# hccho2/Tacotron-Wavenet-Vocoder-Korean

Hardware: AMD Instinct MI355X
Metric: WaveNet autoregressive audio samples/sec at 24 kHz, batch=8 (higher is better)
Workload: dtype f32

## Files before the change

tacotron-wavenet-vocoder-korean_amd/csrc/twv_wavenet_xcd.hip:

```cpp
#include <hip/hip_runtime.h>
#include <stdint.h>
#include <string>
#include <type_traits>
#include "../../include/twv_amd.h"
#include "twv_layout.hpp"
#include "twv_math.hpp"
#include "twv_dev.hpp"
#include "twv_dpp.hpp"
#include "twv_categorical.hpp"
#include "twv_xcd.hpp"

using namespace twv;

#ifndef TWV_CHAIN_PAD
#define TWV_CHAIN_PAD 0
#endif
#ifndef TWV_WATCHDOG_LOG2
#define TWV_WATCHDOG_LOG2 21
#endif
#define TWV_STR2(x) #x
#define TWV_STR(x) TWV_STR2(x)
namespace {

typedef __attribute__((address_space(1))) unsigned long long gu64;
#define LDSU64(i) (((__attribute__((address_space(3))) volatile unsigned long long*)lds)[(i)])

typedef unsigned u32x2v __attribute__((ext_vector_type(2)));
typedef unsigned u32x4s __attribute__((ext_vector_type(4)));
constexpr int kAuxLoad = (int)(16u | 0x80000000u), kAuxStore = 0;
#ifndef TWV_XCD_KF
#define TWV_XCD_KF 1
#endif

__device__ __forceinline__ unsigned long long xb_load(rsrc_t rs, int uword, int lword)
{
    asm volatile("" ::: "memory");
    const u32x2v v = __builtin_amdgcn_raw_buffer_load_b64(rs, lword * 8, uword * 8, kAuxLoad);
    return ((unsigned long long)v.y << 32) | (unsigned long long)v.x;
}
__device__ __forceinline__ u32x4s xb_load2(rsrc_t rs, int uword, int lpair)
{
    asm volatile("" ::: "memory");
    return __builtin_amdgcn_raw_buffer_load_b128(rs, lpair * 16, uword * 8, kAuxLoad);
}
template <bool BAR> __device__ __forceinline__ unsigned long long xb_load_t(rsrc_t rs, int uword, int lword)
{
    if (BAR) asm volatile("" ::: "memory");
    return xb_load(rs, uword, lword);
}
__device__ __forceinline__ unsigned long long xbm_load(rsrc_t rs, int uword, int lword) { return xb_load_t<true>(rs, uword, lword); }
__device__ __forceinline__ u32x4s xbm_load2(rsrc_t rs, int uword, int lpair)
{
    asm volatile("" ::: "memory");
    return xb_load2(rs, uword, lpair);
}
__device__ __forceinline__ void xb_store(rsrc_t rs, int uword, int lword, unsigned tag, float v)
{
    __builtin_amdgcn_raw_buffer_store_b64(u32x2v{__float_as_uint(v), tag}, rs, lword * 8, uword * 8, kAuxStore);
    asm volatile("" ::: "memory");
}
__device__ __forceinline__ void xb_store2(rsrc_t rs, int uword, int lane, unsigned tag, float va, float vb)
{
    const u32x4s d = {__float_as_uint(va), tag, __float_as_uint(vb), tag};
    __builtin_amdgcn_raw_buffer_store_b128(d, rs, lane * 16, uword * 8, kAuxStore);
    asm volatile("s_nop 1" ::"v"(d) : "memory");
}
__device__ __forceinline__ unsigned g_tag(unsigned long long q) { return (unsigned)(q >> 32); }
__device__ __forceinline__ float g_val(unsigned long long q) { return __uint_as_float((unsigned)q); }

struct Poll {
    rsrc_t rs;
    int* status;
    int it;
    bool dead;
};
template <bool BAR = false>
__device__ __forceinline__ bool poll_tick(Poll& p, int code)
{
    if (p.dead) return false;
    if (((++p.it) & 63) == 0) {
        if (xb_load_t<BAR>(p.rs, (int)XcdExch::CTRL + 1, 0) != 0ull) { p.dead = true; return false; }
        if (p.it > (1 << TWV_WATCHDOG_LOG2)) {
            atomicMax(p.status, code);
            xb_store(p.rs, (int)XcdExch::CTRL + 1, 0, 1u, 0.0f);
            p.dead = true;
            return false;
        }
    }
    return true;
}
__device__ __forceinline__ void nap_until(unsigned long long target)
{
#pragma nounroll
    for (int i = 0; i < 4096 && __builtin_amdgcn_s_memtime() < target; ++i) __builtin_amdgcn_s_sleep(8);
}

__device__ __forceinline__ unsigned lds_byte_addr_u64(int i)
{
    return (unsigned)(unsigned long)(&((__attribute__((address_space(3))) unsigned long long*)lds)[i]);
}
__device__ __forceinline__ unsigned lds_byte_addr_u32(int i)
{
    return (unsigned)(unsigned long)(&((__attribute__((address_space(3))) unsigned*)lds)[i]);
}
enum { SPIN_EQ = 0, SPIN_GE = 1 };
#define TWV_SPIN_TAIL                 \
    "s_cmp_eq_u64 vcc, exec\n"        \
    "s_cbranch_scc1 2f\n"             \
    "s_sub_u32 %1, %1, 1\n"           \
    "s_cmp_lg_u32 %1, 0\n"            \
    "s_cbranch_scc1 1b\n"             \
    "2:"
template <int CMP>
__device__ __forceinline__ unsigned long long lds_spin_tag(unsigned byte_addr, unsigned tag, unsigned looks, unsigned& left)
{
    unsigned long long q;
    unsigned n;
    if (CMP == SPIN_GE) {
        const unsigned long long need = (unsigned long long)tag << 32;
        asm volatile(
            "s_mov_b32 %1, %4\n"
            "1:\n"
            "ds_read_b64 %0, %2\n"
            "s_waitcnt lgkmcnt(0)\n"
            "v_cmp_le_u64 vcc, %3, %0\n"
            TWV_SPIN_TAIL
            : "=&v"(q), "=&s"(n)
            : "v"(byte_addr), "s"(need), "s"(looks)
            : "vcc", "scc", "memory");
    } else {
        unsigned long long d;
        const unsigned long long want = (unsigned long long)tag;
        asm volatile(
            "s_mov_b32 %1, %5\n"
            "1:\n"
            "ds_read_b64 %0, %3\n"
            "s_waitcnt lgkmcnt(0)\n"
            "v_lshrrev_b64 %2, 32, %0\n"
            "v_cmp_eq_u64 vcc, %4, %2\n"
            TWV_SPIN_TAIL
            : "=&v"(q), "=&s"(n), "=&v"(d)
            : "v"(byte_addr), "s"(want), "s"(looks)
            : "vcc", "scc", "memory");
    }
    left = n;
    return q;
}
__device__ __forceinline__ void lds_spin_count(unsigned byte_addr, unsigned need, unsigned looks, unsigned& left)
{
    unsigned c, n;
    asm volatile(
        "s_mov_b32 %1, %4\n"
        "1:\n"
        "ds_read_b32 %0, %2\n"
        "s_waitcnt lgkmcnt(0)\n"
        "v_cmp_le_u32 vcc, %3, %0\n"
        TWV_SPIN_TAIL
        : "=&v"(c), "=&s"(n)
        : "v"(byte_addr), "s"(need), "s"(looks)
        : "vcc", "scc", "memory");
    left = n;
}
__device__ __forceinline__ unsigned tag_diff_acc(unsigned acc, unsigned got, unsigned tag)
{
    asm("v_xad_u32 %0, %1, %2, %0" : "+v"(acc) : "v"(got), "s"(tag));
    return acc;
}
template <int CMP>
__device__ __forceinline__ unsigned long long xb_spin_tag(rsrc_t rs, int uword, int lword, unsigned tag, unsigned looks, unsigned& left)
{
    unsigned long long q;
    unsigned n;
    if (CMP == SPIN_GE) {
        const unsigned long long need = (unsigned long long)tag << 32;
        asm volatile(
            "s_mov_b32 %1, %6\n"
            "1:\n"
            "buffer_load_dwordx2 %0, %2, %3, %4 offen sc0 sc1\n"
            "s_waitcnt vmcnt(0)\n"
            "v_cmp_le_u64 vcc, %5, %0\n"
            TWV_SPIN_TAIL
            : "=&v"(q), "=&s"(n)
            : "v"(lword * 8), "s"(rs), "s"(uword * 8), "s"(need), "s"(looks)
            : "vcc", "scc", "memory");
    } else {
        unsigned long long d;
        const unsigned long long want = (unsigned long long)tag;
        asm volatile(
            "s_mov_b32 %1, %7\n"
            "1:\n"
            "buffer_load_dwordx2 %0, %3, %4, %5 offen sc0 sc1\n"
            "s_waitcnt vmcnt(0)\n"
            "v_lshrrev_b64 %2, 32, %0\n"
            "v_cmp_eq_u64 vcc, %6, %2\n"
            TWV_SPIN_TAIL
            : "=&v"(q), "=&s"(n), "=&v"(d)
            : "v"(lword * 8), "s"(rs), "s"(uword * 8), "s"(want), "s"(looks)
            : "vcc", "scc", "memory");
    }
    left = n;
    return q;
}

__device__ __forceinline__ int lane_of_z(int k) { return ((k & 2) ? 16 : 0) + 2 * (k >> 2) + (k & 1); }
__device__ __forceinline__ int lane_of_x(int j) { return j < 16 ? j : 16 + j; }

struct ChainRegs { float wc[32]; float bd; };
__device__ __forceinline__ void dot32_dpp_chain_lo(const float (&w)[16], float xa, float init, float (&c)[4])
{
    float c0 = init, c1, c2, c3;
    asm volatile(
        "s_nop 1\n" TWV_ALIGN8
        "v_fmac_f32_dpp %0, %4, %5 row_newbcast:0 row_mask:0xf bank_mask:0xf\n"
        "v_mul_f32_dpp %1, %4, %6 row_newbcast:1 row_mask:0xf bank_mask:0xf\n"
        "v_mul_f32_dpp %2, %4, %7 row_newbcast:2 row_mask:0xf bank_mask:0xf\n"
        "v_mul_f32_dpp %3, %4, %8 row_newbcast:3 row_mask:0xf bank_mask:0xf\n"
        "v_fmac_f32_dpp %0, %4, %9 row_newbcast:4 row_mask:0xf bank_mask:0xf\n"
        "v_fmac_f32_dpp %1, %4, %10 row_newbcast:5 row_mask:0xf bank_mask:0xf\n"
        "v_fmac_f32_dpp %2, %4, %11 row_newbcast:6 row_mask:0xf bank_mask:0xf\n"
        "v_fmac_f32_dpp %3, %4, %12 row_newbcast:7 row_mask:0xf bank_mask:0xf\n"
        "v_fmac_f32_dpp %0, %4, %13 row_newbcast:8 row_mask:0xf bank_mask:0xf\n"
        "v_fmac_f32_dpp %1, %4, %14 row_newbcast:9 row_mask:0xf bank_mask:0xf\n"
        "v_fmac_f32_dpp %2, %4, %15 row_newbcast:10 row_mask:0xf bank_mask:0xf\n"
        "v_fmac_f32_dpp %3, %4, %16 row_newbcast:11 row_mask:0xf bank_mask:0xf\n"
        "v_fmac_f32_dpp %0, %4, %17 row_newbcast:12 row_mask:0xf bank_mask:0xf\n"
        "v_fmac_f32_dpp %1, %4, %18 row_newbcast:13 row_mask:0xf bank_mask:0xf\n"
        "v_fmac_f32_dpp %2, %4, %19 row_newbcast:14 row_mask:0xf bank_mask:0xf\n"
        "v_fmac_f32_dpp %3, %4, %20 row_newbcast:15 row_mask:0xf bank_mask:0xf"
        : "+v"(c0), "=&v"(c1), "=&v"(c2), "=&v"(c3)
        : "v"(xa), "v"(w[0]), "v"(w[1]), "v"(w[2]), "v"(w[3]), "v"(w[4]), "v"(w[5]), "v"(w[6]), "v"(w[7]), "v"(w[8]), "v"(w[9]), "v"(w[10]), "v"(w[11]), "v"(w[12]), "v"(w[13]), "v"(w[14]), "v"(w[15]));
    c[0] = c0; c[1] = c1; c[2] = c2; c[3] = c3;
}
__device__ __forceinline__ float dot32_dpp_chain_hi(const float (&w)[16], float xb, const float (&c)[4])
{
    float c0 = c[0], c1 = c[1], c2 = c[2], c3 = c[3];
    asm volatile(
        TWV_ALIGN8
        "v_fmac_f32_dpp %0, %4, %5 row_newbcast:0 row_mask:0xf bank_mask:0xf\n"
        "v_fmac_f32_dpp %1, %4, %6 row_newbcast:1 row_mask:0xf bank_mask:0xf\n"
        "v_fmac_f32_dpp %2, %4, %7 row_newbcast:2 row_mask:0xf bank_mask:0xf\n"
        "v_fmac_f32_dpp %3, %4, %8 row_newbcast:3 row_mask:0xf bank_mask:0xf\n"
        "v_fmac_f32_dpp %0, %4, %9 row_newbcast:4 row_mask:0xf bank_mask:0xf\n"
        "v_fmac_f32_dpp %1, %4, %10 row_newbcast:5 row_mask:0xf bank_mask:0xf\n"
        "v_fmac_f32_dpp %2, %4, %11 row_newbcast:6 row_mask:0xf bank_mask:0xf\n"
        "v_fmac_f32_dpp %3, %4, %12 row_newbcast:7 row_mask:0xf bank_mask:0xf\n"
        "v_fmac_f32_dpp %0, %4, %13 row_newbcast:8 row_mask:0xf bank_mask:0xf\n"
        "v_fmac_f32_dpp %1, %4, %14 row_newbcast:9 row_mask:0xf bank_mask:0xf\n"
        "v_fmac_f32_dpp %2, %4, %15 row_newbcast:10 row_mask:0xf bank_mask:0xf\n"
        "v_fmac_f32_dpp %3, %4, %16 row_newbcast:11 row_mask:0xf bank_mask:0xf\n"
        "v_fmac_f32_dpp %0, %4, %17 row_newbcast:12 row_mask:0xf bank_mask:0xf\n"
        "v_fmac_f32_dpp %1, %4, %18 row_newbcast:13 row_mask:0xf bank_mask:0xf\n"
        "v_fmac_f32_dpp %2, %4, %19 row_newbcast:14 row_mask:0xf bank_mask:0xf\n"
        "v_fmac_f32_dpp %3, %4, %20 row_newbcast:15 row_mask:0xf bank_mask:0xf"
        : "+v"(c0), "+v"(c1), "+v"(c2), "+v"(c3)
        : "v"(xb), "v"(w[0]), "v"(w[1]), "v"(w[2]), "v"(w[3]), "v"(w[4]), "v"(w[5]), "v"(w[6]), "v"(w[7]), "v"(w[8]), "v"(w[9]), "v"(w[10]), "v"(w[11]), "v"(w[12]), "v"(w[13]), "v"(w[14]), "v"(w[15]));
    return (c0 + c1) + (c2 + c3);
}

#define XSTAMP(cond_, slot_) do { if ((INSTR & 1) && a.prof != nullptr && b == a.prof_stream && t < a.prof_steps && lane == 0 && (cond_)) a.prof[(long long)t * 64 + (slot_)] = wall_clock64(); } while (0)

#define WACC_DECL() unsigned long long wacc_[6] = {0, 0, 0, 0, 0, 0}, w0_ = 0, wt0_ = 0; if (INSTR & 4) wt0_ = __builtin_amdgcn_s_memtime()
#define WACC_T0() do { if (INSTR & 4) w0_ = __builtin_amdgcn_s_memtime(); } while (0)
#define WACC_T1(i_) do { if (INSTR & 4) wacc_[i_] += __builtin_amdgcn_s_memtime() - w0_; } while (0)
constexpr int kTraceStep = 2000;
#define WTRACE(cond_, slot_) do { if ((INSTR & 4) && a.prof != nullptr && t == kTraceStep && (cond_) && lane == 0) a.prof[2048 + (slot_)] = wall_clock64(); } while (0)
#define WACC_OUT(prof_, slot_, wave_) do { if ((INSTR & 4) && (prof_) != nullptr && (slot_) >= 0 && lane == 0) {                 \
        unsigned long long* o_ = (prof_) + (((slot_) * 8 + (wave_)) * 8);                                                        \
        o_[0] = __builtin_amdgcn_s_memtime() - wt0_;                                                                             \
        o_[1] = wacc_[0]; o_[2] = wacc_[1]; o_[3] = wacc_[2]; o_[4] = wacc_[3]; o_[5] = wacc_[4]; o_[6] = wacc_[5]; } } while (0)
#define XMARK(role_, stage_) do { if ((INSTR & 1) && lane == 0) xb_store(rs, (int)XcdExch::MARK + (role_) * 8 + (int)(threadIdx.x >> 6), 0, (unsigned)t + 1u, (float)(stage_)); } while (0)

enum { ROLE_CHAIN = 0, ROLE_SERVICE = 1, ROLE_SKIP0 = 2, ROLE_CONV0 = 10 };
constexpr int kXcdStreamsPerXcd = kXcdStreams / 8;

struct XArgs {
    XcdLaunch p;
    int n_lc_wg, lc_lpw;
    int n_conv1;
    int total_roles;
};

template <int NS> struct XStreams { rsrc_t rs[NS]; int b[NS]; };
__device__ __forceinline__ rsrc_t exch_rsrc(const XcdLaunch& a, int b)
{
    return __builtin_amdgcn_make_buffer_rsrc(a.exch + (long long)b * XcdExch::WORDS, 0, (int)(XcdExch::WORDS * 8), 0x00020000);
}
struct XLazyRs { const XcdLaunch* a; int xcc, ns; __device__ __forceinline__ rsrc_t operator[](int k) const { return exch_rsrc(*a, xcc + 8 * (k < ns ? k : 0)); } };
struct XLazyB { int xcc, ns; __device__ __forceinline__ int operator[](int k) const { return xcc + 8 * (k < ns ? k : 0); } };
template <int NS> struct XStreamsLazy { XLazyRs rs; XLazyB b; };
constexpr int kSkipLdsWords = 32 * 64;
constexpr int kConvLdsFloats = 16 * 64 + 64;

constexpr int kChainLpw = 5;
template <int INSTR, bool ALL, bool FORCED, bool SEG1, bool TWOSEG, int NC, bool ONEHOT = false, bool HEAD = false, bool CONT = false>
__device__ __forceinline__ void chain_role(const XArgs& xa, int b, rsrc_t rs, const unsigned looks)
{
    const XcdLaunch& a = xa.p;
    const Layout& L = a.lay;
    const int w = __builtin_amdgcn_readfirstlane(threadIdx.x >> 6), lane = threadIdx.x & 63;
    const int NL = L.NL, T = a.T;
    const bool use_bias = L.use_bias != 0, has_gc = L.G > 0, has_lc = L.L > 0;
    constexpr bool forced = FORCED;
    constexpr int kLayerWaves = kXcdSeg0Layers / kChainLpw;
    const int l0 = (SEG1 ? kXcdSeg0Layers : 0) + kChainLpw * w;
    const int lw0 = kChainLpw * w;
    const int cap = (HEAD || w >= kLayerWaves) ? 0 : kChainLpw;
    int nl = NL - l0;
    nl = nl < 0 ? 0 : (nl > cap ? cap : nl);
    const int nlc = NC >= 0 ? NC : nl;
    const bool next_has = (l0 + nl < NL);
    constexpr bool head = HEAD;
    const bool to_seg1 = TWOSEG && !SEG1 && w == kLayerWaves - 1 && next_has;
    constexpr bool two_seg = TWOSEG;
    if (nl == 0 && !head) return;
    const int oc = dpp_conv_out(lane), od = dpp_dense_out(lane);
    const ActCoef coef = act_coef(lane >= 32);
    float* stb = a.state + (long long)b * L.state_stride;
    Poll pl{rs, a.status, 0, false};
    constexpr int O_WD = 2048;
    constexpr int O_WH = kXcdChainHalfTiles;

    float wlo[kChainLpw - 1][16], whi[kChainLpw][16], bdi[kChainLpw];
#pragma unroll
    for (int i = 0; i < kChainLpw; ++i) {
        if (!HEAD && i < nl) {
            const f32x4* src = reinterpret_cast<const f32x4*>(a.P + L.off_xl + (long long)(l0 + i) * kXcdXlFloats) + lane;
#pragma unroll
            for (int q = 0; q < 4; ++q) {
                const f32x4 lo = src[q * 64], hi = src[(4 + q) * 64];
                if (i == 0) LDS4((O_WH >> 2) + (w * 4 + q) * 64 + lane) = lo;
                else { wlo[i > 0 ? i - 1 : 0][4 * q] = lo.x; wlo[i > 0 ? i - 1 : 0][4 * q + 1] = lo.y; wlo[i > 0 ? i - 1 : 0][4 * q + 2] = lo.z; wlo[i > 0 ? i - 1 : 0][4 * q + 3] = lo.w; }
                whi[i][4 * q] = hi.x; whi[i][4 * q + 1] = hi.y; whi[i][4 * q + 2] = hi.z; whi[i][4 * q + 3] = hi.w;
            }
#pragma unroll
            for (int q = 0; q < 4; ++q) LDS4((O_WD >> 2) + ((lw0 + i) * 4 + q) * 64 + lane) = src[(8 + q) * 64];
            const f32x4 v = src[12 * 64];
            bdi[i] = dense_bias_init(lane, use_bias ? v.y : 0.0f);
        }
    }
    float wcz[32];
    float ha = 0.0f, hb = 0.0f, first_in = 0.0f, b2v = 0.0f, s_lnl = 0.0f, s_tq = 0.0f, samp = 0.0f;
    float cp[4] = {0.0f, 0.0f, 0.0f, 0.0f};
    int q_prev = 0, q_valid = 0, samp_q = 0, first_q = 0;
    float w0row = 0.0f;
    double u_next = 0.0;
    const int chx = dpp_dense_out(lane);
    const bool sampler = head && !forced;
    const bool is15 = (lane & 15) == 15;
    auto causal_prepare = [&]() {
        const float t1 = __int_as_float(__builtin_amdgcn_update_dpp(0, __float_as_int(ha), 0x101, 0xf, 0xf, true));
        const float b0 = __int_as_float(__builtin_amdgcn_update_dpp(0, __float_as_int(hb), 0x150, 0xf, 0xf, true));
        ha = is15 ? b0 : t1;
        hb = __int_as_float(__builtin_amdgcn_update_dpp(0, __float_as_int(hb), 0x101, 0xf, 0xf, true));
        causal_partial_dpp(wcz, ha, hb, cp);
    };
    auto noise = [&](int t) {
        const float* up = a.uniforms + ((long long)b * T + t) * (L.nr_mix + 1);
        const float u = lane <= L.nr_mix ? up[lane] : 0.5f;
        s_lnl = log_e(-log_e(u));
        const float uu = __shfl(u, L.nr_mix);
        s_tq = log_e(uu) - log_e(1.0f - uu);
    };
    if (head) {
        if constexpr (ONEHOT) {
            const int* meta = reinterpret_cast<const int*>(stb + L.st_meta);
            q_valid = __builtin_amdgcn_readfirstlane(meta[M_PREV_VALID]);
            q_prev = __builtin_amdgcn_readfirstlane(meta[M_QPREV]) & (L.Q - 1);
            w0row = a.P[L.off_causal + (long long)q_prev * 32 + chx];
            if (!forced) first_q = reinterpret_cast<const int*>(a.first_input)[b];
        } else {
            const f32x4* src = reinterpret_cast<const f32x4*>(a.P + L.off_xc) + lane;
#pragma unroll
            for (int q = 0; q < 8; ++q) { const f32x4 v = src[q * 64]; wcz[4 * q] = v.x; wcz[4 * q + 1] = v.y; wcz[4 * q + 2] = v.z; wcz[4 * q + 3] = v.w; }
            ha = stb[L.st_hist + (lane & 15)];
            hb = stb[L.st_hist + 16 + (lane & 15)];
            if (!forced) first_in = reinterpret_cast<const float*>(a.first_input)[b];
            if (sampler && use_bias && lane < L.O) b2v = a.P[L.off_b2 + lane];
            causal_prepare();
        }
    }
    __builtin_amdgcn_s_waitcnt(0);
    asm volatile(".p2align 6\n\t.rept " TWV_STR(TWV_CHAIN_PAD) "\n\ts_nop 0\n\t.endr" ::: "memory");

    float X = 0.0f;
    unsigned long long t_in = 0, in_period = 0, now_in = 0;
    unsigned long long t_tab = 0, tab_period = 0, now_tab = 0;
    for (int t = 0; t < T && !pl.dead; ++t) {
        asm volatile(".p2align 6");
        const unsigned tag = (unsigned)t + 1u;
        if (head) {
            if (forced && t > 0) {
                unsigned left = 0;
                if (two_seg) (void)xb_spin_tag<SPIN_EQ>(rs, (int)XcdExch::DONE, lane, (unsigned)t, looks, left);
                else (void)lds_spin_tag<SPIN_EQ>(lds_byte_addr_u64(8 * 64 + lane), (unsigned)t, looks, left);
                if (__builtin_expect(left == 0, 0)) {
                    pl.it = 0;
                    for (;;) {
                        const unsigned long long q = two_seg ? xb_load(rs, (int)XcdExch::DONE, lane) : LDSU64(8 * 64 + lane);
                        if (__all(g_tag(q) == (unsigned)t)) break;
                        if (!poll_tick(pl, 35)) break;
                        __builtin_amdgcn_s_sleep(2);
                    }
                }
                if (pl.dead) break;
            }
            XSTAMP(true, 0);
            if constexpr (ONEHOT) {
                const int q_raw = forced ? reinterpret_cast<const int*>(a.forced)[(long long)b * T + t] : (t == 0 ? first_q : samp_q);
                const int q_in = __builtin_amdgcn_readfirstlane(q_raw) & (L.Q - 1);
                const float w1row = a.P[L.off_causal + ((long long)L.Q + q_in) * 32 + chx];
                const float x0 = q_valid ? w0row + w1row : w1row;
                LDSU64(0 * 64 + lane) = ((unsigned long long)tag << 32) | (unsigned long long)__float_as_uint(x0);
                XSTAMP(true, 1);
                if (lane == 0) {
                    if (sampler && t > 0) reinterpret_cast<int*>(a.out)[(long long)b * T + t - 1] = samp_q;
                    xb_store(rs, (int)XcdExch::CTRL, 0, tag, 0.0f);
                }
                q_prev = q_in; q_valid = 1;
                w0row = a.P[L.off_causal + (long long)q_in * 32 + chx];
                if (sampler) u_next = reinterpret_cast<const double*>(a.uniforms)[(long long)b * T + t];
            } else {
            const float s_in = forced ? reinterpret_cast<const float*>(a.forced)[(long long)b * T + t] : (t == 0 ? first_in : samp);
            const float c3 = fma_(wcz[31], s_in, cp[3]);
            const float x0 = (cp[0] + cp[1]) + (cp[2] + c3);
            LDSU64(0 * 64 + lane) = ((unsigned long long)tag << 32) | (unsigned long long)__float_as_uint(x0);
            XSTAMP(true, 1);
            if (lane == 0) {
                if (sampler && t > 0) a.out[(long long)b * T + t - 1] = samp;
                xb_store(rs, (int)XcdExch::CTRL, 0, tag, 0.0f);
            }
            hb = is15 ? s_in : hb;
            if (t + 1 < T) causal_prepare();
            if (sampler) noise(t);
            }
            if (sampler) {
                const unsigned long long d = now_tab - t_tab;
                tab_period = (t_tab != 0 && d < (1ull << 18)) ? d : 0;
                t_tab = now_tab;
            }
            __builtin_amdgcn_s_setprio(0);
        }
        XMARK(SEG1 ? 30 : ROLE_CHAIN, 1);
        float pre[kChainLpw] = {0.0f, 0.0f, 0.0f, 0.0f, 0.0f};
        float w0lo[16];
        if (nlc > 0) {
            pl.it = 0;
            for (;;) {
                bool ok = true;
#pragma unroll
                for (int i = 0; i < kChainLpw; ++i) {
                    if (i < nlc) {
                        const unsigned long long qp = xb_load(rs, (int)XcdExch::PG + (l0 + i) * 64, oc);
                        ok = ok && g_tag(qp) == tag;
                        pre[i] = g_val(qp);
                    }
                }
                if (__all(ok)) break;
                if (!poll_tick(pl, 31)) break;
                __builtin_amdgcn_s_sleep(4);
            }
            XSTAMP(!SEG1, 26 + w);
            XMARK(SEG1 ? 30 : ROLE_CHAIN, 2);
            if (in_period) nap_until(t_in + in_period - (in_period >> 4));
            asm volatile("" ::: "memory");
#pragma unroll
            for (int k = 0; k < 4; ++k) {
                const f32x4 v = LDS4((O_WH >> 2) + (w * 4 + k) * 64 + lane);
                w0lo[4 * k] = v.x; w0lo[4 * k + 1] = v.y; w0lo[4 * k + 2] = v.z; w0lo[4 * k + 3] = v.w;
            }
// ... 114 lines not shown
            if (tab_period) nap_until(t_tab + tab_period - (tab_period >> 3));
            __builtin_amdgcn_s_setprio(3);
            const int half = lane >> 5;
            unsigned long long q[8];
            pl.it = 0;
            for (;;) {
                unsigned diff = 0;
#pragma unroll
                for (int k = 0; k < 4; ++k) {
                    const u32x4s d = xb_load2(rs, (int)XcdExch::PT, (half * 4 + k) * 32 + (lane & 31));
                    q[2 * k] = ((unsigned long long)d.y << 32) | d.x;
                    q[2 * k + 1] = ((unsigned long long)d.w << 32) | d.z;
                    diff = tag_diff_acc(tag_diff_acc(diff, d.y, tag), d.w, tag);
                }
                if (__all(diff == 0u)) break;
                if (!poll_tick(pl, 34)) break;
            }
            now_tab = __builtin_amdgcn_s_memtime();
            XSTAMP(true, 18);
            XMARK(SEG1 ? 30 : ROLE_CHAIN, 5);
            float y = g_val(q[0]);
#pragma unroll
            for (int k = 1; k < 8; ++k) y = y + g_val(q[k]);
#pragma unroll
            for (int k = 0; k < 8; ++k) {
                const auto sw = __builtin_amdgcn_permlane32_swap((unsigned)q[k], (unsigned)q[k], false, false);
                y = y + __uint_as_float(sw[1]);
            }
            if (use_bias && lane < L.O) y = y + b2v;
            if ((INSTR & 2) && a.dbg != nullptr && t < a.dbg_steps)
                a.dbg[((long long)b * a.dbg_steps + t) * ((long long)NL * 64 + L.Opad) + (long long)NL * 64 + lane] = y;
            const int nr = L.nr_mix;
            const float lsmin = (float)-32.23619130191664;
            const float e_all = exp_e(y > lsmin ? y : lsmin);
            const float ninf = __uint_as_float(0xff800000u);
            const float gmb = (lane < nr) ? y - s_lnl : ninf;
            float mx = gmb;
            mx = fmaxf(mx, __int_as_float(__builtin_amdgcn_update_dpp(__float_as_int(ninf), __float_as_int(mx), 0x111, 0xf, 0xf, false)));
            mx = fmaxf(mx, __int_as_float(__builtin_amdgcn_update_dpp(__float_as_int(ninf), __float_as_int(mx), 0x112, 0xf, 0xf, false)));
            mx = fmaxf(mx, __int_as_float(__builtin_amdgcn_update_dpp(__float_as_int(ninf), __float_as_int(mx), 0x114, 0xf, 0xf, false)));
            mx = fmaxf(mx, __int_as_float(__builtin_amdgcn_update_dpp(__float_as_int(ninf), __float_as_int(mx), 0x118, 0xf, 0xf, false)));
            const float best = __int_as_float(__builtin_amdgcn_readlane(__float_as_int(mx), 15));
            const unsigned long long hit = __ballot(lane < nr && gmb == best);
            const int k = hit ? (int)__ffsll((long long)hit) - 1 : 0;
            const float mean = __int_as_float(__builtin_amdgcn_readlane(__float_as_int(y), nr + k));
            const float e = __int_as_float(__builtin_amdgcn_readlane(__float_as_int(e_all), 2 * nr + k));
            const float prod = e * s_tq;
            float xs = mean + prod;
            xs = xs > -1.0f ? xs : -1.0f;
            xs = xs < 1.0f ? xs : 1.0f;
            samp = xs;
            XSTAMP(true, 19);
        }
    }

    if (head) {
        if constexpr (ONEHOT) {
            if (lane == 0) {
                if (sampler && !pl.dead && T > 0) reinterpret_cast<int*>(a.out)[(long long)b * T + T - 1] = samp_q;
                int* meta = reinterpret_cast<int*>(stb + L.st_meta);
                meta[M_TABS] = meta[M_TABS] + T;
                meta[M_PREV_VALID] = q_valid;
                meta[M_QPREV] = q_prev;
            }
        } else {
        if (sampler && !pl.dead && T > 0 && lane == 0) a.out[(long long)b * T + T - 1] = samp;
        if (lane < 16) stb[L.st_hist + lane] = ha;
        else if (lane < 32) stb[L.st_hist + lane] = hb;
        if (lane == 0) {
            int* meta = reinterpret_cast<int*>(stb + L.st_meta);
            meta[M_TABS] = meta[M_TABS] + T;
        }
        }
    }
}

#define TWV_FMAC16_DPP(c0, c1, c2, c3, x, w)                                                          \
    asm volatile(                                                                                      \
        "s_nop 1\n" TWV_ALIGN8                                                                         \
        "v_fmac_f32_dpp %0, %4, %5 row_newbcast:0 row_mask:0xf bank_mask:0xf\n"                        \
        "v_fmac_f32_dpp %1, %4, %6 row_newbcast:1 row_mask:0xf bank_mask:0xf\n"                        \
        "v_fmac_f32_dpp %2, %4, %7 row_newbcast:2 row_mask:0xf bank_mask:0xf\n"                        \
        "v_fmac_f32_dpp %3, %4, %8 row_newbcast:3 row_mask:0xf bank_mask:0xf\n"                        \
        "v_fmac_f32_dpp %0, %4, %9 row_newbcast:4 row_mask:0xf bank_mask:0xf\n"                        \
        "v_fmac_f32_dpp %1, %4, %10 row_newbcast:5 row_mask:0xf bank_mask:0xf\n"                       \
        "v_fmac_f32_dpp %2, %4, %11 row_newbcast:6 row_mask:0xf bank_mask:0xf\n"                       \
        "v_fmac_f32_dpp %3, %4, %12 row_newbcast:7 row_mask:0xf bank_mask:0xf\n"                       \
        "v_fmac_f32_dpp %0, %4, %13 row_newbcast:8 row_mask:0xf bank_mask:0xf\n"                       \
        "v_fmac_f32_dpp %1, %4, %14 row_newbcast:9 row_mask:0xf bank_mask:0xf\n"                       \
        "v_fmac_f32_dpp %2, %4, %15 row_newbcast:10 row_mask:0xf bank_mask:0xf\n"                      \
        "v_fmac_f32_dpp %3, %4, %16 row_newbcast:11 row_mask:0xf bank_mask:0xf\n"                      \
        "v_fmac_f32_dpp %0, %4, %17 row_newbcast:12 row_mask:0xf bank_mask:0xf\n"                      \
        "v_fmac_f32_dpp %1, %4, %18 row_newbcast:13 row_mask:0xf bank_mask:0xf\n"                      \
        "v_fmac_f32_dpp %2, %4, %19 row_newbcast:14 row_mask:0xf bank_mask:0xf\n"                      \
        "v_fmac_f32_dpp %3, %4, %20 row_newbcast:15 row_mask:0xf bank_mask:0xf"                        \
        : "+v"(c0), "+v"(c1), "+v"(c2), "+v"(c3)                                                       \
        : "v"(x), "v"(w[0]), "v"(w[1]), "v"(w[2]), "v"(w[3]), "v"(w[4]), "v"(w[5]), "v"(w[6]), "v"(w[7]), "v"(w[8]), "v"(w[9]), \
          "v"(w[10]), "v"(w[11]), "v"(w[12]), "v"(w[13]), "v"(w[14]), "v"(w[15]))
__device__ __forceinline__ float dot32_dpp_lds(int off4, int lane, float xa, float xb)
{
    float c0 = 0.0f, c1 = 0.0f, c2 = 0.0f, c3 = 0.0f;
#pragma unroll
    for (int h = 0; h < 2; ++h) {
        float w[16];
#pragma unroll
        for (int kq = 0; kq < 4; ++kq) {
            const f32x4 q = LDS4(off4 + (4 * h + kq) * 64 + lane);
            w[4 * kq + 0] = q.x; w[4 * kq + 1] = q.y; w[4 * kq + 2] = q.z; w[4 * kq + 3] = q.w;
        }
        if (h == 0) { TWV_FMAC16_DPP(c0, c1, c2, c3, xa, w); }
        else { TWV_FMAC16_DPP(c0, c1, c2, c3, xb, w); }
    }
    return (c0 + c1) + (c2 + c3);
}
__device__ __forceinline__ void copy_tile_to_lds(int off4, const float* base, int lane)
{
    const f32x4* p = reinterpret_cast<const f32x4*>(base) + lane;
#pragma unroll
    for (int kq = 0; kq < 8; ++kq) LDS4(off4 + kq * 64 + lane) = p[kq * 64];
}

__device__ __forceinline__ unsigned ring_slot(unsigned pos0, unsigned t, unsigned d)
{
    const unsigned v = pos0 + t;
    return (d & (d - 1)) == 0 ? (v & (d - 1)) : v % d;
}
template <int INSTR, bool BIG>
__device__ __forceinline__ void service_role(const XArgs& xa, int b, rsrc_t rs)
{
    const XcdLaunch& a = xa.p;
    const Layout& L = a.lay;
    const int s = __builtin_amdgcn_readfirstlane(threadIdx.x >> 6), lane = threadIdx.x & 63;
    const int NL = L.NL, T = a.T;
    const bool has_lc = L.L > 0, use_bias = L.use_bias != 0, has_gc = L.G > 0;
    float* stb = a.state + (long long)b * L.state_stride;
    float* ring = stb + L.st_ring;
    const int* pmeta = reinterpret_cast<const int*>(a.P + L.off_meta);
    int* ringpos = reinterpret_cast<int*>(stb + L.st_ringpos);
    Poll pl{rs, a.status, 0, false};
    constexpr int kReg = 4, kLds = BIG ? 3 : 0, kSlots = kReg + kLds;
    const int NLDS = BIG ? (NL > 8 * kReg ? NL - 8 * kReg : 0) : 0;
    int nown = 0, nlds = 0;
#pragma unroll
    for (int i = 0; i < kReg; ++i) if (NLDS + s + 8 * i < NL) nown = i + 1;
#pragma unroll
    for (int j = 0; j < kLds; ++j) if (s + 8 * j < NLDS) nlds = j + 1;
    if (nown == 0 && nlds == 0) return;
    Tile t0[kReg];
    unsigned dil[kSlots], roff[kSlots], pos0[kSlots];
    int lay_of[kSlots];
    float bfg[kSlots], gcv[kSlots];
#pragma unroll
    for (int i = 0; i < kSlots; ++i) {
        dil[i] = 1; roff[i] = 0; pos0[i] = 0; bfg[i] = 0.0f; gcv[i] = 0.0f;
        const bool is_lds = i < kLds;
        const int l = is_lds ? s + 8 * i : NLDS + s + 8 * (i - kLds);
        const bool have = is_lds ? i < nlds : (i - kLds) < nown;
        lay_of[i] = have ? l : -1;
        if (have) {
            const float* src = a.P + L.off_layer0 + (long long)l * L.layer_stride + LayerOff::T0;
            if (is_lds) copy_tile_to_lds(l * (kTile / 4), src, lane);
            else load_tile(t0[i - kLds < 0 ? 0 : i - kLds], src, lane);
            dil[i] = (unsigned)pmeta[l]; roff[i] = (unsigned)pmeta[64 + l]; pos0[i] = (unsigned)ringpos[l];
            if (use_bias) bfg[i] = a.P[L.off_layer0 + (long long)l * L.layer_stride + LayerOff::BFG + lane];
            if (has_gc) gcv[i] = a.cond[XH_WORDS + ((long long)b * NL + l) * 64 + lane];
        }
    }
    auto addend = [&](int i, float pre, float lcv) __attribute__((always_inline)) -> float {
        float v = pre;
        if (use_bias) v = v + bfg[i];
        if (has_gc) v = v + gcv[i];
        if (has_lc) v = v + lcv;
        return v;
    };
    const int n16 = lane & 15;
    auto tap0 = [&](int i, unsigned t, float& xa_, float& xb_) __attribute__((always_inline)) {
        const unsigned slot = ring_slot(pos0[i], t, dil[i]);
        const unsigned long long* p = reinterpret_cast<const unsigned long long*>(ring + roff[i] + slot * 32);
        const unsigned long long qa = __hip_atomic_load((gu64*)(p + (n16 >> 1)), __ATOMIC_RELAXED, __HIP_MEMORY_SCOPE_AGENT);
        const unsigned long long qb = __hip_atomic_load((gu64*)(p + 8 + (n16 >> 1)), __ATOMIC_RELAXED, __HIP_MEMORY_SCOPE_AGENT);
        xa_ = __uint_as_float((n16 & 1) ? (unsigned)(qa >> 32) : (unsigned)qa);
        xb_ = __uint_as_float((n16 & 1) ? (unsigned)(qb >> 32) : (unsigned)qb);
    };
    auto dot_slot = [&](int i, float oa, float ob) __attribute__((always_inline)) -> float {
        if (i < kLds) return dot32_dpp_lds(lay_of[i] * (kTile / 4), lane, oa, ob);
        return dot32_dpp(t0[i - kLds < 0 ? 0 : i - kLds].w, oa, ob);
    };
#pragma unroll
    for (int i = 0; i < kSlots; ++i) {
        if (lay_of[i] >= 0) {
            const int l = lay_of[i];
            float xa_, xb_;
            tap0(i, 0u, xa_, xb_);
            const float pre = dot_slot(i, xa_, xb_);
            const float lcv = has_lc ? stb[L.st_lcprev + l * 64 + lane] : 0.0f;
            xb_store(rs, (int)XcdExch::PG + l * 64, lane, 1u, addend(i, pre, lcv));
        }
    }
    for (int t = 0; t < T && !pl.dead; ++t) {
        asm volatile(".p2align 6");
        const unsigned tag = (unsigned)t + 1u;
#pragma unroll
        for (int i = 0; i < kSlots; ++i) {
            if (lay_of[i] >= 0 && !pl.dead) {
                const int l = lay_of[i];
                const bool more = t + 1 < T;
                float oa = 0.0f, ob = 0.0f;
                if (more && dil[i] > 1) tap0(i, (unsigned)t + 1u, oa, ob);
                XMARK(ROLE_SERVICE, 10 + i);
                unsigned long long qa, qb;
                pl.it = 0;
                for (;;) {
                    qa = xb_load(rs, (int)XcdExch::ZX + l * 128 + 1, n16 * 2);
                    qb = xb_load(rs, (int)XcdExch::ZX + l * 128 + 65, n16 * 2);
                    if (__all(g_tag(qa) == tag && g_tag(qb) == tag)) break;
                    if (!poll_tick(pl, 41)) break;
                    __builtin_amdgcn_s_sleep(8);
                }
                if (pl.dead) break;
                const float xa_ = g_val(qa), xb_ = g_val(qb);
                const unsigned slot = ring_slot(pos0[i], (unsigned)t, dil[i]);
                if (lane < 32) ring[roff[i] + slot * 32 + lane] = lane < 16 ? xa_ : xb_;
                if (more) {
                    if (dil[i] == 1) { oa = xa_; ob = xb_; }
                    const float pre = dot_slot(i, oa, ob);
                    float lcv = 0.0f;
                    XMARK(ROLE_SERVICE, 20 + i);
                    if (has_lc) {
                        const int lw = (int)XcdExch::LCR + (((t + 1) % kXcdLcRing) * kXcdLs + l) * 64;
                        unsigned long long ql;
                        pl.it = 0;
                        for (;;) {
                            ql = xb_load(rs, lw, lane);
                            if (__all(g_tag(ql) == tag + 1u)) break;
                            if (!poll_tick(pl, 42)) break;
                            __builtin_amdgcn_s_sleep(8);
                        }
                        if (pl.dead) break;
                        lcv = g_val(ql);
                    }
                    xb_store(rs, (int)XcdExch::PG + l * 64, lane, tag + 1u, addend(i, pre, lcv));
                }
            }
        }
    }
    if (lane == 0 && !pl.dead) {
#pragma unroll
        for (int i = 0; i < kSlots; ++i)
            if (lay_of[i] >= 0) ringpos[lay_of[i]] = (int)((pos0[i] + (unsigned)T) % dil[i]);
    }
}

template <int INSTR, int NS, bool BIG, int KF = 0>
__device__ __forceinline__ void skip_role(const XArgs& xa, const XStreams<NS>& sx, int g, const unsigned looks)
{
    const XcdLaunch& a = xa.p;
    const Layout& L = a.lay;
    const int v = __builtin_amdgcn_readfirstlane(threadIdx.x >> 6), lane = threadIdx.x & 63;
    const int NL = L.NL - KF, T = a.T;
    const bool use_bias = L.use_bias != 0;
    Poll pl{sx.rs[0], a.status, 0, false};
    constexpr int kReg = BIG ? 5 : 4, kLds = BIG ? 2 : 0, kSlots = kReg + kLds;
    const int NLDS = BIG ? (NL > 8 * kReg ? NL - 8 * kReg : 0) : 0;
    const int SW = BIG ? NL * 64 : kSkipLdsWords;
    const int o_tile4 = (NS * SW * 2 + 3) >> 2;
    int nown = 0, nlds = 0;
#pragma unroll
    for (int i = 0; i < kReg; ++i) if (NLDS + v + 8 * i < NL) nown = i + 1;
#pragma unroll
    for (int j = 0; j < kLds; ++j) if (v + 8 * j < NLDS) nlds = j + 1;
    if (nown == 0 && nlds == 0) return;
    Tile ws[kReg];
    float bs[kSlots];
#pragma unroll
    for (int i = 0; i < kSlots; ++i) bs[i] = 0.0f;
#pragma unroll
    for (int i = 0; i < kReg; ++i) {
        if (i < nown) {
            const long long lb = L.off_layer0 + (long long)(NLDS + v + 8 * i) * L.layer_stride;
            load_tile(ws[i], a.P + lb + LayerOff::SK + (long long)g * kTile, lane);
            if (use_bias) bs[kLds + i] = a.P[lb + LayerOff::SK + (long long)L.NSJ * kTile + g * 64 + lane];
        }
    }
#pragma unroll
    for (int j = 0; j < kLds; ++j) {
        if (j < nlds) {
            const long long lb = L.off_layer0 + (long long)(v + 8 * j) * L.layer_stride;
            copy_tile_to_lds(o_tile4 + (v + 8 * j) * (kTile / 4), a.P + lb + LayerOff::SK + (long long)g * kTile, lane);
            if (use_bias) bs[j] = a.P[lb + LayerOff::SK + (long long)L.NSJ * kTile + g * 64 + lane];
        }
    }
    const int n16 = lane & 15;
    const int zc_lane = lane_of_z((lane < 32 ? 0 : 16) + n16);
    unsigned long long seen[kSlots], period = 0;
#pragma unroll
    for (int i = 0; i < kSlots; ++i) seen[i] = 0;
    for (int t = 0; t < T && !pl.dead; ++t) {
        asm volatile(".p2align 6");
        const unsigned tag = (unsigned)t + 1u;
        auto own_layer = [&](auto&& dot, const float bias, const int l, const int si) __attribute__((always_inline)) {
            {
                if (period) nap_until(seen[si] + period - (period >> 3));
                const bool last = l == NL - 1;
                const int lp = l > 0 ? l - 1 : 0;
#pragma unroll
                for (int k = 0; k < NS; ++k) {
                    if (pl.dead) break;
                    const rsrc_t rs = sx.rs[k];
                    const int b = sx.b[k];
                    pl.rs = rs;
                    XMARK(ROLE_SKIP0 + g, 10 + si);
                    unsigned long long qz, qp = 0;
                    pl.it = 0;
                    if (last) {
                        unsigned left = 0;
                        qz = xb_spin_tag<SPIN_EQ>(rs, (int)XcdExch::ZX + l * 128, zc_lane * 2, tag, looks, left);
                        if (__builtin_expect(left == 0, 0)) {
                            pl.it = 0;
                            for (;;) {
                                qz = xb_load(rs, (int)XcdExch::ZX + l * 128, zc_lane * 2);
                                if (__all(g_tag(qz) == tag)) break;
                                if (!poll_tick(pl, 51)) break;
                            }
                        }
                        qp = LDSU64(k * SW + lp * 64 + lane);
                    } else
                    for (;;) {
                        qz = xb_load(rs, (int)XcdExch::ZX + l * 128, zc_lane * 2);
                        qp = LDSU64(k * SW + lp * 64 + lane);
                        if (__all(g_tag(qz) == tag)) break;
                        if (!poll_tick(pl, 51)) break;
                        __builtin_amdgcn_s_sleep(1);
                    }
                    if ((INSTR & 1) && pl.dead && g == 0 && lane == 0) {
                        xb_store(rs, (int)XcdExch::MARK + 176 + v * 4, 0, g_tag(qz), __uint_as_float(g_tag(qz)));
                        xb_store(rs, (int)XcdExch::MARK + 177 + v * 4, 0, (unsigned)l, __uint_as_float((unsigned)pl.it));
                        xb_store(rs, (int)XcdExch::MARK + 178 + v * 4, 0, tag, __uint_as_float((unsigned)si));
                    }
                    XSTAMP(g == 0 && last, 20);
                    const auto sw = __builtin_amdgcn_permlane32_swap((unsigned)qz, (unsigned)qz, false, false);
                    float val = dot(__uint_as_float(sw[0]), __uint_as_float(sw[1]));
                    if (use_bias) val = val + bias;
                    float tot = val;
                    if (l > 0) {
                        asm volatile("" : "+v"(val));
                        if (!__all(g_tag(qp) == tag)) {
                            unsigned left = 0;
                            qp = lds_spin_tag<SPIN_GE>(lds_byte_addr_u64(k * SW + lp * 64 + lane), tag, looks, left);
                            if (left == 0) {
                                pl.it = 0;
                                while (!__all(g_tag(qp) == tag)) {
                                    if (!poll_tick(pl, 52)) break;
                                    qp = LDSU64(k * SW + lp * 64 + lane);
                                }
                            }
                        }
                        tot = g_val(qp) + val;
                    }
                    if (pl.dead) break;
                    if (last) {
                        const float h = (KF > 0 || tot > 0.0f) ? tot : 0.0f;
                        xb_store(rs, (int)XcdExch::H1 + g * 64, lane, tag, h);
                        XSTAMP(g == 0, 21);
                    } else {
                        LDSU64(k * SW + l * 64 + lane) = ((unsigned long long)tag << 32) | (unsigned long long)__float_as_uint(tot);
                    }
                    if (k == 0) {
                        const unsigned long long now = __builtin_amdgcn_s_memtime();
                        if (si == 0) { const unsigned long long d = now - seen[0]; period = (seen[0] != 0 && d < (1ull << 18)) ? d : 0; }
                        seen[si] = now;
                    }
                }
            }
        };
#pragma unroll
        for (int j = 0; j < kLds; ++j) {
            if (j < nlds && !pl.dead)
                own_layer([&](float xa_, float xb_) __attribute__((always_inline)) { return dot32_dpp_lds(o_tile4 + (v + 8 * j) * (kTile / 4), lane, xa_, xb_); }, bs[j], v + 8 * j, j);
        }
#pragma unroll
        for (int i = 0; i < kReg; ++i) {
            if (i < nown && !pl.dead)
                own_layer([&](float xa_, float xb_) __attribute__((always_inline)) { return dot32_dpp(ws[i].w, xa_, xb_); }, bs[kLds + i], NLDS + v + 8 * i, kLds + i);
        }
    }
    if (pl.dead && lane == 0) {
#pragma unroll
        for (int k = 0; k < NS; ++k) xb_store(sx.rs[k], (int)XcdExch::CTRL + 1, 0, 1u, 0.0f);
    }
}

template <int KF, bool BAR>
__device__ __forceinline__ unsigned long long conv1_fetch_h1(Poll& pl, const rsrc_t rs, const int v, const int lane, const unsigned tag, const int last_layer,
                                                             const int zc_lane, const float (&wl)[32], const float bl, const bool use_bias, bool& saw_z, const unsigned looks)
{
    unsigned long long q;
    pl.it = 0;
    if (KF > 0) {
        unsigned long long qz;
        float val = 0.0f;
        for (;;) {
            qz = xb_load_t<BAR>(rs, (int)XcdExch::ZX + last_layer * 128, zc_lane * 2);
            q = xb_load_t<BAR>(rs, (int)XcdExch::H1 + v * 64, lane);
            if (__all(g_tag(qz) == tag)) {
                const auto sw = __builtin_amdgcn_permlane32_swap((unsigned)qz, (unsigned)qz, false, false);
                val = dot32_dpp(wl, __uint_as_float(sw[0]), __uint_as_float(sw[1]));
                if (use_bias) val = val + bl;
                saw_z = true;
                break;
            }
            if (!poll_tick<BAR>(pl, 61)) break;
            __builtin_amdgcn_s_sleep(1);
        }
        if (saw_z && !__all(g_tag(q) == tag)) {
            unsigned left = 0;
            q = xb_spin_tag<SPIN_EQ>(rs, (int)XcdExch::H1 + v * 64, lane, tag, looks, left);
            if (__builtin_expect(left == 0, 0)) {
                pl.it = 0;
                for (;;) {
                    q = xb_load_t<BAR>(rs, (int)XcdExch::H1 + v * 64, lane);
                    if (__all(g_tag(q) == tag)) break;
                    if (!poll_tick<BAR>(pl, 61)) break;
                }
            }
        }
        const float tot = g_val(q) + val;
        const float h = tot > 0.0f ? tot : 0.0f;
        q = (unsigned long long)__float_as_uint(h);
    } else {
        for (;;) {
            q = xb_load_t<BAR>(rs, (int)XcdExch::H1 + v * 64, lane);
            if (__all(g_tag(q) == tag)) break;
            if (!poll_tick<BAR>(pl, 61)) break;
            __builtin_amdgcn_s_sleep(1);
        }
    }
    return q;
}
__device__ __forceinline__ void conv1_load_last_skip(const XcdLaunch& a, const int v, const int lane, Tile& wl, float& bl)
{
    const Layout& L = a.lay;
    const long long lb = L.off_layer0 + (long long)(L.NL - 1) * L.layer_stride;
    load_tile(wl, a.P + lb + LayerOff::SK + (long long)v * kTile, lane);
    if (L.use_bias != 0) bl = a.P[lb + LayerOff::SK + (long long)L.NSJ * kTile + v * 64 + lane];
}
__device__ __forceinline__ void load_half_tile(float (&w)[16], const float* base, const int obase, const int lane)
{
    const float2* p = reinterpret_cast<const float2*>(base + (obase + dpp_dense_out(lane)) * 4 + (((lane >> 4) & 1) ? 2 : 0));
#pragma unroll
    for (int j = 0; j < 8; ++j) {
        const float2 q = p[j * 128];
        w[2 * j] = q.x; w[2 * j + 1] = q.y;
    }
}
__device__ __forceinline__ float conv1d2_chunk_dpp(const float (&t2)[16], const float h)
{
    const float s = dot16_dpp(t2, h);
    const auto ds = __builtin_amdgcn_permlane16_swap(__float_as_uint(s), __float_as_uint(s), false, false);
    return __uint_as_float(ds[0]) + __uint_as_float(ds[1]);
}

template <int INSTR, int NS, bool BAR = false, class SX = XStreams<NS>, int KF = 0>
__device__ __forceinline__ void conv1_role(const XArgs& xa, const SX& sx, int g, const int ns_rt, const int prof_slot, const unsigned looks)
{
    const XcdLaunch& a = xa.p;
    const Layout& L = a.lay;
    const int v = __builtin_amdgcn_readfirstlane(threadIdx.x >> 6), lane = threadIdx.x & 63;
    const int T = a.T, NCH = L.NCH;
    const bool use_bias = L.use_bias != 0;
    Poll pl{sx.rs[0], a.status, 0, false};
    constexpr int O_PART = 0, O_CNT = 16 * 64;
    if (threadIdx.x < NS) LDSI(threadIdx.x * kConvLdsFloats + O_CNT) = 0;
    __syncthreads();
    const int c0 = 2 * v, c1 = 2 * v + 1;
    Tile ta, tb;
    load_tile(ta, a.P + L.off_w1 + ((long long)g * NCH + c0) * kTile, lane);
    load_tile(tb, a.P + L.off_w1 + ((long long)g * NCH + c1) * kTile, lane);
    const bool summer = v < 2;
    const int hz = 32 * v + dpp_z_index(lane);
    float b1v = 0.0f;
    float t2[16];
    if (summer) {
        if (use_bias) b1v = a.P[L.off_b1 + g * 64 + hz];
        load_half_tile(t2, a.P + L.off_w2 + (long long)(2 * g + v) * kTile, 0, lane);
    }
    Tile wl;
    float bl = 0.0f;
    if (KF > 0) conv1_load_last_skip(a, v, lane, wl, bl);
    const int zc_lane = lane_of_z((lane < 32 ? 0 : 16) + (lane & 15));
    unsigned long long t_arr = 0, period = 0;
    WACC_DECL();
    for (int t = 0; t < T && !pl.dead; ++t) {
        asm volatile(".p2align 6");
        const unsigned tag = (unsigned)t + 1u;
        WACC_T0();
        if (period) nap_until(t_arr + period - (period >> 3));
        WACC_T1(0);
#pragma unroll
        for (int k = 0; k < NS; ++k) {
            if (pl.dead) break;
            if (k >= ns_rt) break;
            const rsrc_t rs = sx.rs[k];
            const int b = sx.b[k];
            const int ob = k * kConvLdsFloats;
            pl.rs = rs;
            XMARK(ROLE_CONV0 + g, 1);
            WACC_T0();
            bool saw_z = false;
            const unsigned long long q = conv1_fetch_h1<KF, BAR>(pl, rs, v, lane, tag, L.NL - 1, zc_lane, wl.w, bl, use_bias, saw_z, looks);
            (void)saw_z;
            WACC_T1(1);
            WTRACE(prof_slot >= 0 && k == 0, 400 + g * 8 + v);
            unsigned long long now_arr = 0;
            if (k == 0) now_arr = __builtin_amdgcn_s_memtime();
            XSTAMP(g == 0 && v == 0, 22);
            const unsigned hq = (unsigned)q;
            const auto p16 = __builtin_amdgcn_permlane16_swap(hq, hq, false, false);
            const auto pa = __builtin_amdgcn_permlane32_swap(p16[0], p16[0], false, false);
            const auto pb = __builtin_amdgcn_permlane32_swap(p16[1], p16[1], false, false);
            float r0, r1;
            dot32_dpp_x2(ta.w, __uint_as_float(pa[0]), __uint_as_float(pb[0]), tb.w, __uint_as_float(pa[1]), __uint_as_float(pb[1]), r0, r1);
            lds[ob + O_PART + c0 * 64 + lane] = r0;
            lds[ob + O_PART + c1 * 64 + lane] = r1;
            asm volatile("" ::: "memory");
            if (lane == 0) __hip_atomic_fetch_add(&LDSI(ob + O_CNT), 1, __ATOMIC_RELAXED, __HIP_MEMORY_SCOPE_WORKGROUP);
            if (k == 0) {
                const unsigned long long d = now_arr - t_arr;
                period = (t_arr != 0 && d < (1ull << 18)) ? d : 0;
                t_arr = now_arr;
            }
            XSTAMP(g == 0 && v == 0, 23);
            XMARK(ROLE_CONV0 + g, 2);
            if (summer) {
                WACC_T0();
                unsigned left = 0;
                if (!BAR) lds_spin_count(lds_byte_addr_u32(ob + O_CNT), 8u * tag, looks, left);
                if (__builtin_expect(left == 0, 0)) {
                    pl.it = 0;
                    while (LDSVI(ob + O_CNT) < 8 * (t + 1)) { if (!poll_tick<BAR>(pl, 62)) break; }
                }
                WACC_T1(2);
                asm volatile("" ::: "memory");
                XSTAMP(g == 0 && v == 0, 24);
                float cp[16];
#pragma unroll
                for (int ch = 0; ch < 16; ++ch) cp[ch] = lds[ob + O_PART + ch * 64 + hz];
                __builtin_amdgcn_sched_barrier(0);
                float r = cp[0];
#pragma unroll
                for (int ch = 1; ch < 16; ++ch) r = r + cp[ch];
                if (use_bias) r = r + b1v;
                const float h = r > 0.0f ? r : 0.0f;
                const float p = conv1d2_chunk_dpp(t2, h);
                if ((lane & 16) == 0) xb_store(rs, (int)XcdExch::PT, (g * 32 + dpp_dense_out(lane)) * 2 + v, tag, p);
                WTRACE(prof_slot >= 0 && k == 0, 480 + g * 2 + v);
                XSTAMP(g == 0 && v == 0, 25);
            }
        }
    }
    if (pl.dead && lane == 0) {
#pragma unroll
        for (int k = 0; k < NS; ++k) xb_store(sx.rs[k], (int)XcdExch::CTRL + 1, 0, 1u, 0.0f);
    }
    WACC_OUT(a.prof, prof_slot, v);
}

template <int INSTR, int KF>
__device__ __forceinline__ void conv1_half_role(const XArgs& xa, const XStreams<1>& sx, const int g, const int hh, const unsigned looks)
{
    static_assert(KF > 0, "the last layer's skip 1x1 runs here");
    const XcdLaunch& a = xa.p;
    const Layout& L = a.lay;
    const int v = __builtin_amdgcn_readfirstlane(threadIdx.x >> 6), lane = threadIdx.x & 63;
    const int T = a.T, NCH = L.NCH;
    const bool use_bias = L.use_bias != 0;
    const rsrc_t rs = sx.rs[0];
    const int b = sx.b[0];
    Poll pl{rs, a.status, 0, false};
    constexpr int O_PART = 0, O_CNT = 16 * 64;
    if (threadIdx.x == 0) LDSI(O_CNT) = 0;
    __syncthreads();
    const int c0 = 2 * v, c1 = 2 * v + 1;
    float ta[16], tb[16];
    load_half_tile(ta, a.P + L.off_w1 + ((long long)g * NCH + c0) * kTile, 32 * hh, lane);
    load_half_tile(tb, a.P + L.off_w1 + ((long long)g * NCH + c1) * kTile, 32 * hh, lane);
    const int zi = dpp_z_index(lane), od = dpp_dense_out(lane);
    const int hl = 32 * (lane >> 5) + zi;
    const bool summer = v == 0;
    float b1v = 0.0f;
    float t2[16];
    if (summer) {
        if (use_bias) b1v = a.P[L.off_b1 + g * 64 + 32 * hh + zi];
        load_half_tile(t2, a.P + L.off_w2 + (long long)(2 * g + hh) * kTile, 0, lane);
    }
    Tile wl;
    float bl = 0.0f;
    conv1_load_last_skip(a, v, hl, wl, bl);
    const int zc_lane = lane_of_z((lane < 32 ? 0 : 16) + (lane & 15));
    unsigned long long t_arr = 0, period = 0;
    for (int t = 0; t < T && !pl.dead; ++t) {
        asm volatile(".p2align 6");
        const unsigned tag = (unsigned)t + 1u;
        if (period) nap_until(t_arr + period - (period >> 3));
        XMARK(ROLE_CONV0 + 2 * g + hh, 1);
        bool saw_z = false;
        const unsigned long long q = conv1_fetch_h1<KF, false>(pl, rs, v, hl, tag, L.NL - 1, zc_lane, wl.w, bl, use_bias, saw_z, looks);
        (void)saw_z;
        const unsigned long long now_arr = __builtin_amdgcn_s_memtime();
        XSTAMP(g == 0 && hh == 0 && v == 0, 22);
        const unsigned hq = (unsigned)q;
        const auto hs = __builtin_amdgcn_permlane32_swap(hq, hq, false, false);
        float s0, s1;
        dot16_dpp_x2(ta, __uint_as_float(hs[0]), tb, __uint_as_float(hs[1]), s0, s1);
        const auto d0 = __builtin_amdgcn_permlane16_swap(__float_as_uint(s0), __float_as_uint(s0), false, false);
        const auto d1 = __builtin_amdgcn_permlane16_swap(__float_as_uint(s1), __float_as_uint(s1), false, false);
        const float r0 = __uint_as_float(d0[0]) + __uint_as_float(d0[1]);
        const float r1 = __uint_as_float(d1[0]) + __uint_as_float(d1[1]);
        if ((lane & 16) == 0) {
            lds[O_PART + c0 * 32 + od] = r0;
            lds[O_PART + c1 * 32 + od] = r1;
        }
        asm volatile("" ::: "memory");
        if (lane == 0) __hip_atomic_fetch_add(&LDSI(O_CNT), 1, __ATOMIC_RELAXED, __HIP_MEMORY_SCOPE_WORKGROUP);
        {
            const unsigned long long d = now_arr - t_arr;
            period = (t_arr != 0 && d < (1ull << 18)) ? d : 0;
            t_arr = now_arr;
        }
        XSTAMP(g == 0 && hh == 0 && v == 0, 23);
        XMARK(ROLE_CONV0 + 2 * g + hh, 2);
        if (summer) {
            unsigned left = 0;
            lds_spin_count(lds_byte_addr_u32(O_CNT), 8u * tag, looks, left);
            if (__builtin_expect(left == 0, 0)) {
                pl.it = 0;
                while (LDSVI(O_CNT) < 8 * (t + 1)) { if (!poll_tick(pl, 62)) break; }
            }
            asm volatile("" ::: "memory");
            XSTAMP(g == 0 && hh == 0, 24);
            float cp[16];
#pragma unroll
            for (int ch = 0; ch < 16; ++ch) cp[ch] = lds[O_PART + ch * 32 + zi];
            __builtin_amdgcn_sched_barrier(0);
            float r = cp[0];
#pragma unroll
            for (int ch = 1; ch < 16; ++ch) r = r + cp[ch];
            if (use_bias) r = r + b1v;
            const float h = r > 0.0f ? r : 0.0f;
            const float p = conv1d2_chunk_dpp(t2, h);
            if ((lane & 16) == 0) xb_store(rs, (int)XcdExch::PT, (g * 32 + od) * 2 + hh, tag, p);
            XSTAMP(g == 0 && hh == 0, 25);
        }
    }
    if (pl.dead && lane == 0) xb_store(rs, (int)XcdExch::CTRL + 1, 0, 1u, 0.0f);
}

constexpr int kConvQLdsFloats = 16 * 64 + 64 + 8 * 64;
template <int INSTR, int NS, int KF = 0>
__device__ __forceinline__ void conv1_onehot_role(const XArgs& xa, const XStreams<NS>& sx, int g, const unsigned looks)
{
    const XcdLaunch& a = xa.p;
    const Layout& L = a.lay;
    const int v = __builtin_amdgcn_readfirstlane(threadIdx.x >> 6), lane = threadIdx.x & 63;
    const int T = a.T, NCH = L.NCH;
    const bool use_bias = L.use_bias != 0;
    Poll pl{sx.rs[0], a.status, 0, false};
    constexpr int O_PART = 0, O_CNT = 16 * 64, O_P2 = 16 * 64 + 64;
    if (threadIdx.x < NS) { LDSI(threadIdx.x * kConvQLdsFloats + O_CNT) = 0; LDSI(threadIdx.x * kConvQLdsFloats + O_CNT + 1) = 0; }
// ... 1362 lines not shown
```

Measured before the change: 1.036 million.

## Break serial per-layer skip-sum chain into segments reduced at segment ends

Previously every layer waited on the previous layer's LDS partial before adding its own dot product, so the per-sample latency was a serial chain across all layers. Now each layer inside a segment of kChainLpw layers publishes only its own contribution. The segment-end layer (or the last layer) waits on all of that segment's tagged partials plus the previous segment's total, then sums them. This shortens the cross-wave dependency chain, at the cost of polling several LDS tags per wait and a changed floating-point summation order. It also adds instrumentation stamps for segment boundaries, and the helpers hardcode five slots, so they assume kChainLpw equals five.

After: 1.043 million (median of 6 runs). About the same (+0.7%).

```diff
diff --git a/tacotron-wavenet-vocoder-korean_amd/csrc/twv_wavenet_xcd.hip b/tacotron-wavenet-vocoder-korean_amd/csrc/twv_wavenet_xcd.hip
--- a/tacotron-wavenet-vocoder-korean_amd/csrc/twv_wavenet_xcd.hip
+++ b/tacotron-wavenet-vocoder-korean_amd/csrc/twv_wavenet_xcd.hip
@@ -165,6 +165,23 @@
 {
     asm("v_xad_u32 %0, %1, %2, %0" : "+v"(acc) : "v"(got), "s"(tag));
     return acc;
+}
+__device__ __forceinline__ void lds_load_tags(const int w0, unsigned long long (&q)[5])
+{
+#pragma unroll
+    for (int j = 0; j < 5; ++j) q[j] = LDSU64(w0 + 64 * j);
+}
+__device__ __forceinline__ bool lds_test_tags(const unsigned long long (&q)[5], const int nv, const unsigned tag)
+{
+    unsigned acc = 0u;
+#pragma unroll
+    for (int j = 0; j < 5; ++j) acc = tag_diff_acc(acc, j < nv ? g_tag(q[j]) : tag, tag);
+    return __all(acc == 0u);
+}
+__device__ __forceinline__ bool lds_look_tags(const int w0, const int nv, const unsigned tag, unsigned long long (&q)[5])
+{
+    lds_load_tags(w0, q);
+    return lds_test_tags(q, nv, tag);
 }
 template <int CMP>
 __device__ __forceinline__ unsigned long long xb_spin_tag(rsrc_t rs, int uword, int lword, unsigned tag, unsigned looks, unsigned& left)
@@ -885,7 +902,16 @@
             {
                 if (period) nap_until(seen[si] + period - (period >> 3));
                 const bool last = l == NL - 1;
-                const int lp = l > 0 ? l - 1 : 0;
+                int lx = l;
+                asm volatile("" : "+s"(lx));
+                const int lm = lx % kChainLpw;
+                const bool seg_end = last || lm == kChainLpw - 1;
+                const int lo = lx > lm ? lx - lm - 1 : 0;
+                const int nw = seg_end ? l - lo : 0;
+                const int wb = l >= kChainLpw ? lx - kChainLpw : 0;
+                const int nv = l >= kChainLpw ? kChainLpw : l;
+                const int seg_j = lx / kChainLpw - ((NL + kChainLpw - 1) / kChainLpw - 5);
+                const bool seg_stamp = (INSTR & 1) && g == 0 && !last && lm == kChainLpw - 1 && seg_j >= 0 && seg_j < 4;
 #pragma unroll
                 for (int k = 0; k < NS; ++k) {
                     if (pl.dead) break;
@@ -893,7 +919,11 @@
                     const int b = sx.b[k];
                     pl.rs = rs;
                     XMARK(ROLE_SKIP0 + g, 10 + si);
-                    unsigned long long qz, qp = 0;
+                    unsigned long long qz, qs[kChainLpw];
+#pragma unroll
+                    for (int j = 0; j < kChainLpw; ++j) qs[j] = 0;
+                    const int wq = k * SW + wb * 64 + lane;
+                    bool have = false;
                     pl.it = 0;
                     if (last) {
                         unsigned left = 0;
@@ -906,11 +936,11 @@
                                 if (!poll_tick(pl, 51)) break;
                             }
                         }
-                        qp = LDSU64(k * SW + lp * 64 + lane);
+                        if (nw > 0) lds_load_tags(wq, qs);
                     } else
                     for (;;) {
                         qz = xb_load(rs, (int)XcdExch::ZX + l * 128, zc_lane * 2);
-                        qp = LDSU64(k * SW + lp * 64 + lane);
+                        if (nw > 0) lds_load_tags(wq, qs);
                         if (__all(g_tag(qz) == tag)) break;
                         if (!poll_tick(pl, 51)) break;
                         __builtin_amdgcn_s_sleep(1);
@@ -921,24 +951,29 @@
                         xb_store(rs, (int)XcdExch::MARK + 178 + v * 4, 0, tag, __uint_as_float((unsigned)si));
                     }
                     XSTAMP(g == 0 && last, 20);
+                    XSTAMP(seg_stamp, 56 + 2 * seg_j);
                     const auto sw = __builtin_amdgcn_permlane32_swap((unsigned)qz, (unsigned)qz, false, false);
                     float val = dot(__uint_as_float(sw[0]), __uint_as_float(sw[1]));
                     if (use_bias) val = val + bias;
                     float tot = val;
-                    if (l > 0) {
+                    if (nw > 0) {
                         asm volatile("" : "+v"(val));
-                        if (!__all(g_tag(qp) == tag)) {
-                            unsigned left = 0;
-                            qp = lds_spin_tag<SPIN_GE>(lds_byte_addr_u64(k * SW + lp * 64 + lane), tag, looks, left);
-                            if (left == 0) {
+                        have = lds_test_tags(qs, nv, tag);
+                        if (!have) {
+                            unsigned left = looks;
+                            do { have = lds_look_tags(wq, nv, tag, qs); } while (!have && --left != 0u);
+                            if (__builtin_expect(!have, 0)) {
                                 pl.it = 0;
-                                while (!__all(g_tag(qp) == tag)) {
-                                    if (!poll_tick(pl, 52)) break;
-                                    qp = LDSU64(k * SW + lp * 64 + lane);
+                                for (;;) {
+                                    if (lds_look_tags(wq, nv, tag, qs)) break;
+                                    if (!poll_tick(pl, 54)) break;
                                 }
                             }
                         }
-                        tot = g_val(qp) + val;
+                        tot = -0.0f;
+#pragma unroll
+                        for (int j = 0; j < kChainLpw; ++j) tot = tot + (wb + j >= lo && wb + j < l ? g_val(qs[j]) : -0.0f);
+                        tot = tot + val;
                     }
                     if (pl.dead) break;
                     if (last) {
@@ -947,6 +982,7 @@
                         XSTAMP(g == 0, 21);
                     } else {
                         LDSU64(k * SW + l * 64 + lane) = ((unsigned long long)tag << 32) | (unsigned long long)__float_as_uint(tot);
+                        XSTAMP(seg_stamp, 57 + 2 * seg_j);
                     }
                     if (k == 0) {
                         const unsigned long long now = __builtin_amdgcn_s_memtime();
```
